# MiguelAlgaba/photoconsistency-visual-odometry

Measured on AMD Instinct MI355X. Metric: frame-pair alignments/sec (640x480, 4-level), higher is better.
Workload: dtype f64

## Files before the change

photoconsistency-visual-odometry_amd/csrc/gn_device.hpp:

```cpp
#pragma once

#include <hip/hip_runtime.h>
#include <hip/hip_fp16.h>

#include "phovo_internal.hpp"

namespace phovo_hip {

namespace {

constexpr int WAVE = 64;
constexpr size_t LDS_LIMIT = 160 * 1024;
constexpr int NRED = 32;
constexpr int RED_VALID = 27;

enum {
  C_X = 0, C_Y, C_Z, C_R01, C_R02, C_R11, C_R12,
  C_T1, C_T2, C_T3, C_T4, C_T5, C_T6, C_T8, C_T11, C_T14, C_T15,
  C_T16, C_T17, C_T24, C_CY, C_SY, C_COUNT
};

enum { CTL_DONE = 0, CTL_FLAGS = 1, CTL_PAIR = 2, CTL_OOW = 3, CTL_COUNT = 4 };

__host__ __device__ constexpr size_t lds_fixed_bytes(int threads)
// ... 399 lines not shown
  s.hi_step_r1 = __double2hiint((double)(step_r + 1));
  return s;
}
__device__ __forceinline__ void rowcol_advance(double &cd, double &rd, const RowColStep &s)
{
  cd += s.step_c;
  const bool wrap = cd >= s.w;
  cd -= __hiloint2double(wrap ? s.hi_w : 0, 0);
  rd += __hiloint2double(wrap ? s.hi_step_r1 : s.hi_step_r, 0);
}

struct RowColFromIndex {
  double inv_w, half_inv_w, w;
};
__device__ __forceinline__ RowColFromIndex make_rowcol_from_index(int W)
{
  RowColFromIndex m;
  m.w = (double)W;
  m.inv_w = uniform_f64(1.0 / m.w);
  m.half_inv_w = 0.5 * m.inv_w;
  return m;
}
__device__ __forceinline__ void rowcol_from_index(double kd, const RowColFromIndex &m, double &cd, double &rd)
{
  rd = trunc(fma(kd, m.inv_w, m.half_inv_w));
  cd = fma(-rd, m.w, kd);
}

__device__ __forceinline__ void rowcol_from_index_floor(double kd, const RowColFromIndex &m, double &cd, double &rd)
{
  rd = floor(fma(kd, m.inv_w, m.half_inv_w));
  cd = fma(-rd, m.w, kd);
}

__device__ __forceinline__ double wave_butterfly(double (&acc)[NRED], int lane)
{
  reduce_stage_swap<32, false>(acc);
  reduce_stage_swap<16, true>(acc);
  reduce_stage<8, 4, 8>(acc, lane);
  reduce_stage<4, 4, 4>(acc, lane);
  reduce_stage<2, 4, 2>(acc, lane);
  return acc[0] + dpp_f64<DPP_QUAD_XOR1>(acc[0]);
}

__device__ __forceinline__ void reduce_wave_to_row(double (&acc)[NRED], int lane, int row, double *s_red)
{
  const double total = wave_butterfly(acc, lane);
  const int idx = ((lane >> 5) & 1) * 16 + ((lane >> 4) & 1) * 8 + ((lane >> 3) & 1) * 4 +
                  ((lane >> 2) & 1) * 2 + ((lane >> 1) & 1);
  if ((lane & 1) == 0) s_red[row * NRED + idx] = total;
}

template <int NROWS>
__device__ __forceinline__ void sum_rows_broadcast(int lane, double *s_red, double (&h)[21], double (&g)[6], int &n_valid)
{
  static_assert(NROWS == 1 || NROWS % 2 == 0, "the rows are summed in two halves");
  if constexpr (NROWS > 1) {
    const int j = lane & (NRED - 1);
    const int w0 = (lane >> 5) * (NROWS / 2);
    double r[NROWS / 2];
#pragma unroll
    for (int w2 = 0; w2 < NROWS / 2; w2++) r[w2] = s_red[(w0 + w2) * NRED + j];
    double v = 0.0;
#pragma unroll
    for (int w2 = 0; w2 < NROWS / 2; w2++) v += r[w2];
    const unsigned vlo = (unsigned)__double2loint(v), vhi = (unsigned)__double2hiint(v);
    const auto lo = __builtin_amdgcn_permlane32_swap(vlo, vlo, false, false);
    const auto hi = __builtin_amdgcn_permlane32_swap(vhi, vhi, false, false);
    v = __hiloint2double((int)hi[0], (int)lo[0]) + __hiloint2double((int)hi[1], (int)lo[1]);
    if (lane < NRED) s_red[lane] = v;
  }
#pragma unroll
  for (int q = 0; q < 21; q++) h[q] = s_red[q];
#pragma unroll
  for (int i = 0; i < 6; i++) g[i] = s_red[21 + i];
  n_valid = (int)s_red[RED_VALID];
}

template <int N>
__device__ __forceinline__ void update_and_terminate(int lane, const double (&step)[N], const double (&g)[N], double *s_state,
                                                     double *s_cst, int *s_ctl, double lambda, int max_iter,
                                                     double min_grad_norm, int iteration, int last_valid, double &last_gnorm)
{
  double st[N];
  bool finite = true;
#pragma unroll
  for (int i = 0; i < N; i++) {
    st[i] = s_state[i] - lambda * step[i];
    finite = finite && finite_f64(st[i]);
  }
  double gn2 = 0.0;
#pragma unroll
  for (int i = 0; i < N; i++) gn2 += g[i] * g[i];
  const double gnorm = sqrt(gn2);
  bool done = false;
  if (iteration + 1 >= max_iter) done = true;
  else if (gnorm < min_grad_norm) done = true;
  if (!finite) done = true;
  if (!done) write_pose_constants(st[0], st[1], st[2], st[3], st[4], st[5], s_cst, lane);
  if (lane == 0) {
#pragma unroll
    for (int i = 0; i < N; i++) s_state[i] = st[i];
    s_ctl[CTL_DONE] = done ? 1 : 0;
    if (!finite) s_ctl[CTL_FLAGS] |= (int)PHOVO_PAIR_NONFINITE;
    if (last_valid < N) s_ctl[CTL_FLAGS] |= (int)PHOVO_PAIR_RANK_DEFICIENT;
  }
  last_gnorm = gnorm;
}

template <int NROWS>
__device__ __forceinline__ void sum_rows_solve_update(int lane, double *s_red, double *s_state, double *s_cst, int *s_ctl,
                                                      double lambda, int max_iter, double min_grad_norm,
                                                      int iteration, double &last_gnorm, int &last_valid)
{
  double h[21], g[6];
  sum_rows_broadcast<NROWS>(lane, s_red, h, g, last_valid);
  double step[6];
  solve6_ldlt(h, g, step);
  update_and_terminate<6>(lane, step, g, s_state, s_cst, s_ctl, lambda, max_iter, min_grad_norm, iteration, last_valid,
                          last_gnorm);
}

template <int NW>
__device__ __forceinline__ void reduce_solve_update(double (&acc)[NRED], int lane, int wave, double *s_red,
                                                    double *s_state, double *s_cst, int *s_ctl,
                                                    double lambda, int max_iter, double min_grad_norm,
                                                    int iteration, double &last_gnorm, int &last_valid)
{
  reduce_wave_to_row(acc, lane, wave, s_red);
  __syncthreads();
  if (wave == 0)
    sum_rows_solve_update<NW>(lane, s_red, s_state, s_cst, s_ctl, lambda, max_iter, min_grad_norm, iteration, last_gnorm,
                              last_valid);
  __syncthreads();
}

__device__ __forceinline__ void add_row(double (&acc)[NRED], const double (&Jw)[6], const double (&J)[6], const double res)
{
  int q = 0;
#pragma unroll
  for (int a = 0; a < 6; a++) {
#pragma unroll
    for (int b = a; b < 6; b++) {
      acc[q] = fma(Jw[a], J[b], acc[q]);
      q++;
    }
  }
#pragma unroll
  for (int a = 0; a < 6; a++) acc[21 + a] = fma(Jw[a], res, acc[21 + a]);
}
__device__ __forceinline__ void add_row(double (&acc)[NRED], const double (&J)[6], const double res) { add_row(acc, J, J, res); }

template <int RCP_STEPS>
__device__ __forceinline__ void analytic_row(const double px, const double py, const double pz, const double gxi, const double gyi,
                                             const double fx, const double fy, const double x, const double y, const double z,
                                             const double t1, const double t2, const double t3, const double t4, const double t5,
                                             const double t6, const double t9, const double t11, const double t14,
                                             const double t15, const double cosy, const double siny, double (&J)[6], double &Zr)
{
  Zr = py * t1 + pz * t2 - px * t3;
  const double t25 = fast_rcp<RCP_STEPS>(z + Zr);
  const double Au = pz * t4 + py * t5 + px * t11;
  const double Bv = fma(py, t6, fma(pz, t9, fma(px, t14, y)));
  J[0] = (gxi * fx) * t25;
  J[1] = (gyi * fy) * t25;
  J[2] = -(J[0] * Au + J[1] * Bv) * t25;
  const double Xr = fma(-px, x, Au);
  const double nYr = y - Bv;
  const double ncx = fma(Zr, J[1], nYr * J[2]);
  const double cyc = fma(Zr, J[0], -(Xr * J[2]));
  J[3] = fma(J[1], Xr, J[0] * nYr);
  J[4] = fma(cosy, cyc, siny * ncx);
  J[5] = fma(-t3, J[3], fma(t14, cyc, -(t15 * ncx)));
}

template <typename Kernel, typename Args>
hipError_t launch_persistent(Kernel kernel, int n_pairs, int cu_count, int wgs_per_cu, int threads, size_t lds_bytes,
                             hipStream_t stream, const Args &args)
{
  const int resident = cu_count * wgs_per_cu;
  const dim3 grid((unsigned)(n_pairs < resident ? n_pairs : resident)), block((unsigned)threads);
  hipLaunchKernelGGL(kernel, grid, block, lds_bytes, stream, args);
  return hipGetLastError();
}

}

}
```

photoconsistency-visual-odometry_amd/csrc/gn_kernels.hip:

```cpp

#include <hip/hip_runtime.h>
#include <hip/hip_fp16.h>

#include <cstdlib>
#include <type_traits>

#include "gn_device.hpp"
#include "phovo_internal.hpp"

namespace phovo_hip {

namespace {

#ifdef PHOVO_TIMELINE
#define PHOVO_TIMELINE_BEGIN const int tl_begin = (int)(wall_clock64() & 0x7fffffffull);
#define PHOVO_TIMELINE_END(rep) { (rep).valid_pixels[15] = tl_begin; (rep).valid_pixels[14] = (int)(wall_clock64() & 0x7fffffffull); (rep).iterations[15] = (int)blockIdx.x; }
#else
#define PHOVO_TIMELINE_BEGIN
#define PHOVO_TIMELINE_END(rep)
#endif

struct LevelLds {
  double *cst;
  double *state;
// ... 75 lines not shown
#define PHOVO_STAMP(i) { const unsigned long long t_ = wall_clock64(); stamp_sum[i] += t_ - stamp_last; stamp_last = t_; }
#else
#define PHOVO_STAMP(i)
#endif
  bool first_trip = true;
  while (true) {
#ifdef PHOVO_PHASE_STAMPS
    stamp_last = wall_clock64();
#endif
    int wv = wave;
    if constexpr (NW > 1) asm volatile("" : "+s"(wv));
    const double fr00 = uniform_f64(s_cst[P_FR00]), fr01 = uniform_f64(s_cst[P_FR01]), fr02 = uniform_f64(s_cst[P_FR02]);
    const double fr10 = uniform_f64(s_cst[P_FR10]), fr11 = uniform_f64(s_cst[P_FR11]), fr12 = uniform_f64(s_cst[P_FR12]);
    const double t1 = uniform_f64(s_cst[P_T1]), t2 = uniform_f64(s_cst[P_T2]), t3 = uniform_f64(s_cst[P_T3]);
    const double cxv = s_cst[P_XF], cyv = s_cst[P_YF], czv = s_cst[P_Z];
    const double oxv = s_cst[P_OXI], oyv = s_cst[P_OYI];

    int owner_tag = 0;
    if constexpr (!OWNER_LDS) {
      const int tg = iteration % OWNER_TAG_PERIOD + 1;
      if (iteration > 0 && tg == 1) {
        for (int kk = n_lds + tid; kk < n; kk += T) g_owner[kk] = -1;
        asm volatile("s_waitcnt vmcnt(0) lgkmcnt(0)" ::: "memory");
        __syncthreads();
      }
      owner_tag = tg << OWNER_TAG_SHIFT;
    }

    int inb_lo = 0, inb_hi = 0;
    int n_rows = 0;
    {
      int k = k0, j = 0;
      PHOVO_ROWCOL_BEGIN
      double pz_next;
      if (PARK && OWNER_LDS && !first_trip && wv < depth_chunks) pz_next = s_i0[k];
      else pz_next = plane_load<TD>(rS, k, oD);
      auto warp_chunk = [&](const double pz, const int chunk, unsigned long long &m_out, int &t_out) {
        PHOVO_ROWCOL_HERE
        const double px = fma(cd, ifx, oxv) * pz;
        const double py = fma(rd, ify, oyv) * pz;
        const double Xf = fma(fr02, pz, fma(fr01, py, fma(fr00, px, cxv)));
        const double Yf = fma(fr12, pz, fma(fr11, py, fma(fr10, px, cyv)));
        const double Z = fma(t2, pz, fma(t1, py, fma(-t3, px, czv)));
        const double iz = fast_rcp(Z);
        const double tc = fma(Xf, iz, ox);
        const double tr = fma(Yf, iz, oy);
        const double half_below = __hiloint2double(0x3fdfffff, (int)0xffffffff);
        const int ri = __double2int_rz(tr + half_below), ci = __double2int_rz(tc + half_below);
        const int lanes_left = n - chunk * WAVE;
        const unsigned long long in_image = lanes_left >= WAVE ? ~0ull : ((1ull << lanes_left) - 1ull);
        const unsigned long long m =
            in_image & __builtin_amdgcn_ballot_w64(min_d < pz) &
            __builtin_amdgcn_ballot_w64(pz < max_d) & __builtin_amdgcn_ballot_w64(tr > -0.5) &
            __builtin_amdgcn_ballot_w64(ri < H) & __builtin_amdgcn_ballot_w64(tc > -0.5) &
            __builtin_amdgcn_ballot_w64(ci < W);
        m_out = m;
        t_out = mad24_uniform_b(ri, W, ci);
      };
      auto keep_mask = [&](const unsigned long long m, const int chunk) {
        if (!MASK_REG) n_rows += __builtin_popcountll(m);
        if (MASK_REG) {
          inb_lo = writelane_b32(inb_lo, (int)(unsigned)m, j);
          inb_hi = writelane_b32(inb_hi, (int)(unsigned)(m >> 32), j);
        } else {
          if (lane == 0) s_mask[chunk] = m;
        }
      };
      if constexpr (OWNER_LDS) {
        auto chunk_body = [&](const int chunk, auto next_parked_tag, auto park_tag) {
          const double pz = pz_next;
          if constexpr (decltype(next_parked_tag)::value) pz_next = s_i0[k + NW * WAVE];
          else pz_next = plane_load<TD>(rS, k + NW * WAVE, oD);
          if constexpr (decltype(park_tag)::value) {
            if (chunk < depth_chunks) s_i0[k] = pz;
          }
          unsigned long long m;
          int t;
          warp_chunk(pz, chunk, m, t);
          if (__builtin_amdgcn_inverse_ballot_w64(m)) atomicMax(&s_owner[t], k);
          keep_mask(m, chunk);
          k += NW * WAVE;
          j++;
          PHOVO_ROWCOL_NEXT
        };
        if (!PARK || first_trip) {
          int chunk = wv;
          for (; chunk + NW < A.n_chunks; chunk += 2 * NW) {
            chunk_body(chunk, std::false_type{}, std::bool_constant<PARK>{});
            chunk_body(chunk + NW, std::false_type{}, std::bool_constant<PARK>{});
          }
          if (chunk < A.n_chunks) chunk_body(chunk, std::false_type{}, std::bool_constant<PARK>{});
        } else {
          const int my_chunks = wv < A.n_chunks ? (A.n_chunks - 1 - wv) / NW + 1 : 0;
          const int parked = depth_chunks > wv ? min(my_chunks, (depth_chunks - 1 - wv) / NW + 1) : 0;
          auto run = [&](int c_lo, int c_end, auto tag) {
            int c = c_lo;
            for (; c + 1 < c_end; c += 2) {
              chunk_body(wv + c * NW, tag, std::false_type{});
              chunk_body(wv + (c + 1) * NW, tag, std::false_type{});
            }
            if (c < c_end) chunk_body(wv + c * NW, tag, std::false_type{});
          };
          if (parked > 0) {
            run(0, parked - 1, std::true_type{});
            chunk_body(wv + (parked - 1) * NW, std::false_type{}, std::false_type{});
          }
          run(parked, my_chunks, std::false_type{});
        }
      } else {
        constexpr int G = 4;
        double pzg[G], pzn[G];
        int pend_t[G], pend_v[G];
        unsigned long long pend_m[G];
        pzg[0] = pz_next;
#pragma unroll
        for (int g = 1; g < G; g++) pzg[g] = plane_load<TD>(rS, k + g * NW * WAVE, oD);
        int chunk = wv;
        while (chunk < A.n_chunks) {
#pragma unroll
          for (int g = 0; g < G; g++) pzn[g] = plane_load<TD>(rS, k + (G + g) * NW * WAVE, oD);
          int count = 0;
#pragma unroll
          for (int g = 0; g < G; g++) {
            if (chunk < A.n_chunks) {
              warp_chunk(pzg[g], chunk, pend_m[g], pend_t[g]);
              pend_v[g] = owner_tag | k;
              keep_mask(pend_m[g], chunk);
              count = g + 1;
              chunk += NW;
              k += NW * WAVE;
              j++;
              PHOVO_ROWCOL_NEXT
            }
          }
#pragma unroll
          for (int g = 0; g < G; g++) {
            if (g < count && __builtin_amdgcn_inverse_ballot_w64(pend_m[g])) {
              if (pend_t[g] < n_lds) atomicMax(&s_owner[pend_t[g]], pend_v[g] & OWNER_INDEX_MASK);
              else atomicMax(&g_owner[pend_t[g]], pend_v[g]);
            }
          }
#pragma unroll
          for (int g = 0; g < G; g++) pzg[g] = pzn[g];
        }
      }
    }
    PHOVO_STAMP(0)
    __syncthreads();
    PHOVO_STAMP(1)

    const double cz = uniform_f64(s_cst[P_Z]), cx = uniform_f64(s_cst[P_X]);
    const double t4 = uniform_f64(s_cst[P_T4]), t5 = uniform_f64(s_cst[P_T5]), t6 = uniform_f64(s_cst[P_T6]);
    const double t8 = uniform_f64(s_cst[P_T8]), t11 = uniform_f64(s_cst[P_T11]), t14 = uniform_f64(s_cst[P_T14]);
    const double t15 = uniform_f64(s_cst[P_T15]);
    const double cosy = uniform_f64(s_cst[P_CY]), siny = uniform_f64(s_cst[P_SY]);
    const double t9 = -t8;

    double acc[NRED];
#pragma unroll
    for (int j = 0; j < NRED; j++) acc[j] = 0.0;

    auto pass2 = [&](auto huber_tag) {
      constexpr bool HUBER = decltype(huber_tag)::value;
      constexpr bool REV = OWNER_LDS;
      const int my_chunks = wv < A.n_chunks ? (A.n_chunks - 1 - wv) / NW + 1 : 0;
      const int first = REV ? my_chunks - 1 : 0;
      const int k_step = REV ? -NW * WAVE : NW * WAVE;
      int k = k0 + first * (NW * WAVE), j = first;
      double kd = kd0 + (double)first * kd_step, cd, rd;
      int o_n = -1;
      double pz_n = 0.0, gx_n = 0.0, gy_n = 0.0, i1_n = 0.0, i0_n = 0.0;
      const double oxv2 = s_cst[P_OXI], oyv2 = s_cst[P_OYI], cyv2 = s_cst[P_Y];
      int o_raw = -1;
      auto owner_request = [&](int kk) {
        o_raw = (kk >= n_lds && kk < n) ? __hip_atomic_load(&g_owner[kk], __ATOMIC_RELAXED, __HIP_MEMORY_SCOPE_AGENT) : -1;
      };
      if (!OWNER_LDS) owner_request(k);
      int o_ahead = -1;
      auto fetch = [&](int kk, auto parked_tag, const bool another_behind) {
        o_n = -1;
        if (OWNER_LDS) {
          o_n = o_ahead;
          o_ahead = -1;
          if (another_behind) {
            const int k2 = kk + k_step;
            o_ahead = s_owner[k2];
            s_owner[k2] = -1;
          }
        } else {
          if (kk < n_lds) {
            o_n = s_owner[kk];
            s_owner[kk] = -1;
          } else {
            o_n = (o_raw & ~OWNER_INDEX_MASK) == owner_tag ? (o_raw & OWNER_INDEX_MASK) : -1;
          }
          owner_request(kk + NW * WAVE);
        }
        if constexpr (decltype(parked_tag)::value) pz_n = s_i0[max(kk, 0)];
        else pz_n = plane_load<TD>(rS, kk, oD);
        gx_n = plane_load<TI>(rT, kk, oGX);
        gy_n = plane_load<TI>(rT, kk, oGY);
        i1_n = plane_load<TI>(rT, kk, oI);
        if (SRC_LDS) { if (o_n >= 0) i0_n = s_i0[o_n]; }
        else i0_n = plane_load<TI>(rS, o_n, oI);
      };
      if (OWNER_LDS && my_chunks > 0) {
        o_ahead = s_owner[k];
        s_owner[k] = -1;
      }
      if (PARK && wv + first * NW < depth_chunks) fetch(k, std::true_type{}, my_chunks >= 2);
      else fetch(k, std::false_type{}, my_chunks >= 2);
      auto chunk_body = [&](const int chunk, auto next_parked_tag, const int behind) {
        const int o = o_n;
        const double pz = pz_n, gxi = gx_n, gyi = gy_n, pixel2 = i1_n, pixel1 = i0_n;
        fetch(k + k_step, next_parked_tag, behind > 0);
        const unsigned long long mbits =
            MASK_REG ? (((unsigned long long)(unsigned)__builtin_amdgcn_readlane(inb_hi, j) << 32) |
                        (unsigned long long)(unsigned)__builtin_amdgcn_readlane(inb_lo, j))
                     : s_mask[chunk];
        if (__builtin_amdgcn_inverse_ballot_w64(mbits)) {
          const double res = (o >= 0) ? (pixel2 - pixel1) : 0.0;
          PHOVO_ROWCOL_HERE
          const double px = fma(cd, ifx, oxv2) * pz;
          const double py = fma(rd, ify, oyv2) * pz;

          double J[6], Zr;
          analytic_row<1>(px, py, pz, gxi, gyi, fx, fy, cx, cyv2, cz, t1, t2, t3, t4, t5, t6, t9, t11, t14, t15, cosy, siny, J, Zr);

          double Jw[6];
#pragma unroll
          for (int a = 0; a < 6; a++) Jw[a] = J[a];
          if (HUBER) {
            const double ar = fabs(res);
            const double wgt = ar <= huber_delta ? 1.0 : huber_delta / ar;
#pragma unroll
            for (int a = 0; a < 6; a++) Jw[a] = J[a] * wgt;
          }
          int q = 0;
#pragma unroll
          for (int a = 0; a < 6; a++) {
#pragma unroll
            for (int b = a; b < 6; b++) {
              acc[q] = fma(Jw[a], J[b], acc[q]);
              q++;
            }
          }
#pragma unroll
          for (int a = 0; a < 6; a++) acc[21 + a] = fma(Jw[a], res, acc[21 + a]);
        }
        k += k_step;
        j += REV ? -1 : 1;
        kd += REV ? -kd_step : kd_step;
      };
      if (REV) {
        auto run = [&](int c_hi, int c_lo, auto tag) {
          for (int c = c_hi; c >= c_lo; c -= 2) {
            chunk_body(wv + c * NW, tag, c - 1);
            if (c > c_lo) chunk_body(wv + (c - 1) * NW, tag, c - 2);
          }
        };
        if (PARK) {
          const int c_split = depth_chunks > wv ? min(my_chunks - 1, (depth_chunks - 1 - wv) / NW + 1) : -1;
          run(my_chunks - 1, c_split + 1, std::false_type{});
          run(min(my_chunks - 1, c_split), 0, std::true_type{});
        } else {
          run(my_chunks - 1, 0, std::false_type{});
        }
      } else {
        for (int chunk = wv; chunk < A.n_chunks; chunk += 2 * NW) {
          chunk_body(chunk, std::false_type{}, 0);
          if (chunk + NW < A.n_chunks) chunk_body(chunk + NW, std::false_type{}, 0);
        }
      }
    };
    if (huber_on) pass2(std::true_type{}); else pass2(std::false_type{});
    PHOVO_STAMP(2)
    acc[RED_VALID] = MASK_REG ? (double)(__popc((unsigned)inb_lo) + __popc((unsigned)inb_hi)) : (lane == 0 ? (double)n_rows : 0.0);


    {
      const double total = wave_butterfly(acc, lane);
      int ln = lane;
      asm volatile("" : "+v"(ln));
      const int idx = ((ln >> 5) & 1) * 16 + ((ln >> 4) & 1) * 8 + ((ln >> 3) & 1) * 4 + ((ln >> 2) & 1) * 2 + ((ln >> 1) & 1);
      if ((ln & 1) == 0) s_red[wave * NRED + idx] = total;
    }
    PHOVO_STAMP(3)
    __syncthreads();
    PHOVO_STAMP(4)

    if (wave == 0) {
      int ln0 = lane;
      asm volatile("" : "+v"(ln0));
      double h[21], g[6];
      sum_rows_broadcast<NW>(ln0, s_red, h, g, last_valid);
#ifdef PHOVO_PHASE_STAMPS
      asm volatile("" :: "v"(h[0]), "v"(g[5]));
      const unsigned long long solve_t0 = wall_clock64();
#endif
      double step[6];
      solve6_ldlt(h, g, step);
#ifdef PHOVO_PHASE_STAMPS
      asm volatile("" :: "v"(step[0]), "v"(step[5]));
      const unsigned long long solve_t1 = wall_clock64();
      solve_sum[0] += solve_t0 - stamp_last;
      solve_sum[1] += solve_t1 - solve_t0;
#endif
      double st[6];
      bool finite = true;
#pragma unroll
      for (int i = 0; i < 6; i++) {
        st[i] = s_state[i] - A.lambda * step[i];
        finite = finite && (fabs(st[i]) <= 1.79769313486231570815e308);
      }
      double gn2 = 0.0;
#pragma unroll
      for (int i = 0; i < 6; i++) gn2 += g[i] * g[i];
      const double gnorm = sqrt(gn2);
      const int it = iteration + 1;
      bool done = false;
      if (it >= A.max_iter) done = true;
      else if (gnorm < A.min_grad_norm) done = true;
      if (!finite) done = true;
#ifdef PHOVO_PHASE_STAMPS
      asm volatile("" :: "v"(gnorm));
      const unsigned long long solve_t2 = wall_clock64();
      solve_sum[2] += solve_t2 - solve_t1;
#endif
      if (!done) write_pass_constants(st[0], st[1], st[2], st[3], st[4], st[5], fx, fy, s_cst, lane);
#ifdef PHOVO_PHASE_STAMPS
      asm volatile("s_waitcnt lgkmcnt(0)" ::: "memory");
      solve_sum[3] += wall_clock64() - solve_t2;
#endif
      if (lane == 0) {
#pragma unroll
        for (int i = 0; i < 6; i++) s_state[i] = st[i];
        s_ctl[CTL_DONE] = done ? 1 : 0;
        if (!finite) s_ctl[CTL_FLAGS] |= (int)PHOVO_PAIR_NONFINITE;
        if (last_valid < 6) s_ctl[CTL_FLAGS] |= (int)PHOVO_PAIR_RANK_DEFICIENT;
      }
      last_gnorm = gnorm;
    }
    __syncthreads();
    PHOVO_STAMP(5)
    iteration++;
    first_trip = false;
    if (s_ctl[CTL_DONE]) break;
  }
#ifdef PHOVO_PHASE_STAMPS
  if (blockIdx.x == 0 && lane == 0 && (wave == 0 || wave == 1 || wave == NW / 2 || wave == NW - 1))
    printf("stamps T=%d level n=%d it=%d wave %2d: pass1 %llu barrier %llu pass2 %llu butterfly %llu barrier %llu solve/wait %llu prologue %llu (10 ns ticks)\n",
           T, n, iteration, wave, stamp_sum[0], stamp_sum[1], stamp_sum[2], stamp_sum[3], stamp_sum[4], stamp_sum[5], stamp_prologue);
  if (blockIdx.x == 0 && lane == 0 && wave == 0)
    printf("stamps T=%d level n=%d it=%d inside wave 0's serial section: row sums %llu  LDL^T %llu  update+norm %llu  pose constants %llu\n",
           T, n, iteration, solve_sum[0], solve_sum[1], solve_sum[2], solve_sum[3]);
#endif
#undef PHOVO_STAMP
#undef PHOVO_ROWCOL_BEGIN
#undef PHOVO_ROWCOL_HERE
#undef PHOVO_ROWCOL_NEXT
}


template <int T, bool SRC_LDS, bool OWNER_LDS, bool MASK_REG>
__device__ __forceinline__ LevelLds carve_lds(unsigned char *lds_raw, int n_max, int n_chunks_max)
{
  constexpr int NW = T / WAVE;
  LevelLds L;
  L.cst = reinterpret_cast<double *>(lds_raw);
  L.state = L.cst + 32;
  L.red = L.state + 8;
  L.ctl = reinterpret_cast<int *>(L.red + NW * NRED);
  L.mask = reinterpret_cast<unsigned long long *>(L.ctl + CTL_COUNT);
  unsigned char *p = reinterpret_cast<unsigned char *>(L.mask + (MASK_REG ? 0 : n_chunks_max));
  L.owner = reinterpret_cast<int *>(p);
  if (OWNER_LDS) p += sizeof(int) * (size_t)owner_lds_entries(n_max, T);
  L.i0 = reinterpret_cast<double *>(p);
  return L;
}

template <int T, int WPS, bool SRC_LDS, bool OWNER_LDS, bool MASK_REG, typename TI, typename TD, bool PARK = false>
__global__ __launch_bounds__(T, WPS) __attribute__((aligned(T == WAVE ? 4096 : 256))) void gn_level_kernel(const GNLevelArgs A)
{
  if constexpr (T == WAVE) asm volatile(".fill 896, 4, 0xbf800000");
  extern __shared__ __align__(16) unsigned char lds_raw[];
  const LevelLds L = carve_lds<T, SRC_LDS, OWNER_LDS, MASK_REG>(lds_raw, A.n, A.g_mask ? 0 : A.n_chunks);
  int *const s_ctl = L.ctl;
  const int tid = threadIdx.x;
  for (int k = tid; k < (OWNER_LDS ? owner_lds_entries(A.n, T) : A.n_lds); k += T) L.owner[k] = -1;
  if (tid == 0) s_ctl[CTL_PAIR] = draw_pair_any(A);
  for (;;) {
    asm volatile("s_waitcnt lgkmcnt(0)" ::: "memory");
    __syncthreads();
    const int pair = __builtin_amdgcn_readfirstlane(s_ctl[CTL_PAIR]);
    if (pair >= A.n_pairs) break;

    int iteration = 0;
    if (A.handover_in) iteration = __builtin_amdgcn_readfirstlane(A.reports[pair].iterations[A.level]);
    double last_gnorm = 0.0;
    int last_valid = 0;
    PHOVO_TIMELINE_BEGIN
    level_body<T, SRC_LDS, OWNER_LDS, MASK_REG, TI, TD, PARK>(A, L, pair, false, iteration, last_gnorm, last_valid);

    if (tid == 0) {
#pragma unroll
      for (int j = 0; j < 6; j++) A.states[(size_t)pair * 6 + j] = L.state[j];
      if (A.reports) {
        A.reports[pair].iterations[A.level] = iteration;
        A.reports[pair].gradient_norm = last_gnorm;
        A.reports[pair].valid_pixels[A.level] = last_valid;
        const uint32_t new_flags = (uint32_t)s_ctl[CTL_FLAGS] | (A.handover_in ? A.takeover_flag : 0u);
        if (new_flags) atomicOr(&A.reports[pair].flags, new_flags);
        PHOVO_TIMELINE_END(A.reports[pair])
      }
      s_ctl[CTL_PAIR] = draw_pair_any(A);
    }
  }
}

template <int T, int WPS, typename TI, typename TD>
__global__ __launch_bounds__(T, WPS) void gn_fused_kernel(const GNFusedArgs F)
{
  extern __shared__ __align__(16) unsigned char lds_raw[];
  const LevelLds L = carve_lds<T, false, true, true>(lds_raw, F.n_max, 0);
  int *const s_ctl = L.ctl;
  const int tid = threadIdx.x;
  for (int k = tid; k < owner_lds_entries(F.n_max, T); k += T) L.owner[k] = -1;
  if (tid == 0) s_ctl[CTL_PAIR] = draw_pair(F.work_counter, F.n_queues, F.n_pairs);
  for (;;) {
    asm volatile("s_waitcnt lgkmcnt(0)" ::: "memory");
    __syncthreads();
    const int pair = __builtin_amdgcn_readfirstlane(s_ctl[CTL_PAIR]);
    if (pair >= F.n_pairs) break;

    double last_gnorm = 0.0;
    PHOVO_TIMELINE_BEGIN
    for (int li = 0; li < F.n_levels; li++) {
      const GNLevelArgs &A = F.lv[li];
      int iteration = 0, last_valid = 0;
      LevelLds Ll = L;
      int *const tail = L.owner + owner_lds_entries(A.n, T);
      Ll.i0 = reinterpret_cast<double *>(tail);
      level_body<T, false, true, true, TI, TD, true>(A, Ll, pair, li > 0, iteration, last_gnorm, last_valid);
      for (int k = tid; k < A.depth_lds_chunks * (int)(WAVE * sizeof(double) / sizeof(int)); k += T) tail[k] = -1;
      if (tid == 0 && A.reports) {
        A.reports[pair].iterations[A.level] = iteration;
        A.reports[pair].valid_pixels[A.level] = last_valid;
      }
    }

    if (tid == 0) {
      const GNLevelArgs &A = F.lv[0];
// ... 201 lines not shown
```

photoconsistency-visual-odometry_amd/csrc/gn_slide_kernel.hip:

```cpp
#include <hip/hip_runtime.h>
#include <hip/hip_fp16.h>

#include <cstdlib>
#include <type_traits>

#include "gn_device.hpp"
#include "phovo_internal.hpp"

namespace phovo_hip {

namespace {

constexpr int SLIDE_RING_PX = 32768;
constexpr int SLIDE_MASK_RING = 512;
static_assert((SLIDE_RING_PX & (SLIDE_RING_PX - 1)) == 0 && (SLIDE_MASK_RING & (SLIDE_MASK_RING - 1)) == 0, "ring indices are masks");

template <int T_, int NW1_, int B1_, int B2_>
struct SlideGeom {
  static constexpr int T = T_, NW = T_ / WAVE, NW1 = NW1_, NW2 = NW - NW1_, B1 = B1_, B2 = B2_;
  static constexpr int BAND_CHUNKS = NW1 * B1;
  static constexpr int BAND_PX = BAND_CHUNKS * WAVE;
  static constexpr int RING_BANDS = SLIDE_RING_PX / BAND_PX;
  static constexpr int M_MAX = (RING_BANDS - 1) / 2;
  static_assert(NW1 * B1 == NW2 * B2, "both kinds of waves cover one band per phase");
  static_assert(NW2 % 2 == 0, "the cross-wave sum splits the rows of s_red in two halves");
  static_assert((M_MAX + 2) * BAND_CHUNKS <= SLIDE_MASK_RING, "ballots of the bands between pass 1 and pass 2");
};

template <int T, int NW1, int B1, int B2, typename TI, typename TD>
__global__ __launch_bounds__(T, T / 256) void gn_level_kernel_slide(const GNLevelArgs A)
{
  using G = SlideGeom<T, NW1, B1, B2>;
  constexpr int NW2 = G::NW2, BAND_CHUNKS = G::BAND_CHUNKS, BAND_PX = G::BAND_PX;
  extern __shared__ __align__(16) unsigned char lds_raw[];
  double *s_cst = reinterpret_cast<double *>(lds_raw);
  double *s_state = s_cst + 32;
  double *s_red = s_state + 8;
  int *s_ctl = reinterpret_cast<int *>(s_red + NW2 * NRED);
  unsigned long long *s_mask = reinterpret_cast<unsigned long long *>(s_ctl + CTL_COUNT);
  int *s_owner = reinterpret_cast<int *>(s_mask + SLIDE_MASK_RING);

  const int tid = threadIdx.x;
  const int lane = tid & (WAVE - 1);
  const int wave = __builtin_amdgcn_readfirstlane(tid / WAVE);
  const int n = A.n, W = A.w, H = A.h;
  const int n_bands = (A.n_chunks + BAND_CHUNKS - 1) / BAND_CHUNKS;
  const int m_run = A.slide_m;
  const int n_phases = n_bands + m_run + 1;
  const int oI = (int)A.plane_off[PLANE_I], oD = (int)A.plane_off[PLANE_D];
  const int oGX = (int)A.plane_off[PLANE_GX], oGY = (int)A.plane_off[PLANE_GY];
  if (tid == 0) s_ctl[CTL_PAIR] = draw_pair(A.work_counter, A.n_queues, A.n_pairs);
  for (;;) {
  asm volatile("s_waitcnt lgkmcnt(0)" ::: "memory");
  __syncthreads();
  const int pair = __builtin_amdgcn_readfirstlane(s_ctl[CTL_PAIR]);
  if (pair >= A.n_pairs) break;

  const __amdgpu_buffer_rsrc_t rS = frame_rsrc(A.planes + (size_t)A.src[pair] * A.frame_bytes, A.frame_bytes);
  const __amdgpu_buffer_rsrc_t rT = frame_rsrc(A.planes + (size_t)A.tgt[pair] * A.frame_bytes, A.frame_bytes);

  for (int k = tid; k < SLIDE_RING_PX; k += T) s_owner[k] = -1;
  if (wave == 0) {
    double st[6];
#pragma unroll
    for (int j = 0; j < 6; j++) st[j] = A.states[(size_t)pair * 6 + j];
    write_pose_constants(st[0], st[1], st[2], st[3], st[4], st[5], s_cst, lane);
    if (lane == 0) {
#pragma unroll
      for (int j = 0; j < 6; j++) s_state[j] = st[j];
      s_ctl[CTL_DONE] = 0;
      s_ctl[CTL_FLAGS] = 0;
      s_ctl[CTL_OOW] = 0;
    }
  }
  __syncthreads();

  const double fx = A.fx, fy = A.fy, ox = A.ox, oy = A.oy, ifx = A.ifx, ify = A.ify;
  const double dW = (double)W;
  const double oxi = uniform_f64(-(ox + 0.5) * ifx), oyi = uniform_f64(-oy * ify);
  const double inv_w = uniform_f64(1.0 / dW);

  int iteration = 0;
  double last_gnorm = 0.0;
  int last_valid = 0;
  bool handed_over = false;
  while (true) {
    if (wave < NW1) {
      const double min_d = A.min_depth, max_d = A.max_depth;
      const double cx = uniform_f64(s_cst[C_X]), cyy = uniform_f64(s_cst[C_Y]), cz = uniform_f64(s_cst[C_Z]);
      const double fr00 = uniform_f64(uniform_f64(s_cst[C_T15]) * fx), fr01 = uniform_f64(uniform_f64(s_cst[C_R01]) * fx);
      const double fr02 = uniform_f64(uniform_f64(s_cst[C_R02]) * fx);
      const double fr10 = uniform_f64(uniform_f64(s_cst[C_T14]) * fy), fr11 = uniform_f64(uniform_f64(s_cst[C_R11]) * fy);
      const double fr12 = uniform_f64(uniform_f64(s_cst[C_R12]) * fy);
      const double t1 = uniform_f64(s_cst[C_T1]), t2 = uniform_f64(s_cst[C_T2]), t3 = uniform_f64(s_cst[C_T3]);
      double cxv = cx * fx, cyv = cyy * fy, czv = cz, oxv = oxi, oyv = oyi;
      asm volatile("" : "+v"(cxv), "+v"(cyv), "+v"(czv), "+v"(oxv), "+v"(oyv));
      const double half_below = __hiloint2double(0x3fdfffff, (int)0xffffffff);
      constexpr int STEP = NW1 * WAVE;
      int k1 = wave * WAVE + lane, chunk1 = wave;
      double kd1 = (double)k1 + 0.5;
      double pzb[B1];
#pragma unroll
      for (int b = 0; b < B1; b++) pzb[b] = plane_load<TD>(rS, k1 + b * STEP, oD);
      for (int s = 0; s < n_bands; s++) {
        const int win_lo = (s - m_run + 1) * BAND_PX;
        const unsigned win_span = (unsigned)(2 * m_run * BAND_PX);
#pragma unroll
        for (int b = 0; b < B1; b++) {
          const double pz = pzb[b];
          pzb[b] = plane_load<TD>(rS, k1 + B1 * STEP, oD);
          const double rd = trunc(kd1 * inv_w), cd = fma(-rd, dW, kd1);
          const double px = fma(cd, ifx, oxv) * pz;
          const double py = fma(rd, ify, oyv) * pz;
          const double Xf = fma(fr02, pz, fma(fr01, py, fma(fr00, px, cxv)));
          const double Yf = fma(fr12, pz, fma(fr11, py, fma(fr10, px, cyv)));
          const double Z = fma(t2, pz, fma(t1, py, fma(-t3, px, czv)));
          const double iz = fast_rcp(Z);
          const double tc = fma(Xf, iz, ox);
          const double tr = fma(Yf, iz, oy);
          const int ri = __double2int_rz(tr + half_below), ci = __double2int_rz(tc + half_below);
          const int lanes_left = n - chunk1 * WAVE;
          const unsigned long long in_image =
              lanes_left >= WAVE ? ~0ull : (lanes_left > 0 ? ((1ull << lanes_left) - 1ull) : 0ull);
          unsigned long long m =
              in_image & __builtin_amdgcn_ballot_w64(min_d < pz) & __builtin_amdgcn_ballot_w64(pz < max_d) &
              __builtin_amdgcn_ballot_w64(tr > -0.5) & __builtin_amdgcn_ballot_w64(ri < H) &
              __builtin_amdgcn_ballot_w64(tc > -0.5) & __builtin_amdgcn_ballot_w64(ci < W);
          const int t = mad24_uniform_b(ri, W, ci);
          const unsigned long long inside = __builtin_amdgcn_ballot_w64((unsigned)(t - win_lo) < win_span);
          if (m & ~inside) {
            if (lane == 0) s_ctl[CTL_OOW] = 1;
            m &= inside;
          }
          if (__builtin_amdgcn_inverse_ballot_w64(m)) atomicMax(&s_owner[t & (SLIDE_RING_PX - 1)], k1);
          if (lane == 0) s_mask[chunk1 & (SLIDE_MASK_RING - 1)] = m;
          k1 += STEP;
          chunk1 += NW1;
          kd1 += (double)STEP;
        }
        __syncthreads();
      }
      for (int s = n_bands; s < n_phases; s++) __syncthreads();
    } else {
      const int wave2 = wave - NW1;
      const double cx = uniform_f64(s_cst[C_X]), cyy = uniform_f64(s_cst[C_Y]), cz = uniform_f64(s_cst[C_Z]);
      const double t1 = uniform_f64(s_cst[C_T1]), t2 = uniform_f64(s_cst[C_T2]), t3 = uniform_f64(s_cst[C_T3]);
      const double t14 = uniform_f64(s_cst[C_T14]);
      const double t4 = uniform_f64(s_cst[C_T4]), t5 = uniform_f64(s_cst[C_T5]), t6 = uniform_f64(s_cst[C_T6]);
      const double t8 = uniform_f64(s_cst[C_T8]), t11 = uniform_f64(s_cst[C_T11]);
      const double t15 = uniform_f64(s_cst[C_T15]);
      const double cosy = uniform_f64(s_cst[C_CY]), siny = uniform_f64(s_cst[C_SY]);
      const double t9 = -t8;
      const double huber_delta = A.huber_delta;
      const bool huber_on = huber_delta > 0.0;
      constexpr int STEP = NW2 * WAVE;

      double acc[NRED];
#pragma unroll
      for (int j = 0; j < NRED; j++) acc[j] = 0.0;
      int n_rows = 0;

      for (int s = 0; s < m_run; s++) __syncthreads();
      int k2 = wave2 * WAVE + lane, chunk2 = wave2;
      double kd2 = (double)k2 + 0.5;
      struct Slots {
        int own[B2];
        double i0[B2], pz[B2], gx[B2], gy[B2], i1[B2];
      };
      Slots set_a, set_b;
      auto request = [&](Slots &S, const int b, const int kk) {
        const int o = s_owner[kk & (SLIDE_RING_PX - 1)];
        s_owner[kk & (SLIDE_RING_PX - 1)] = -1;
        S.own[b] = o;
        S.pz[b] = plane_load<TD>(rS, kk, oD);
        S.gx[b] = plane_load<TI>(rT, kk, oGX);
        S.gy[b] = plane_load<TI>(rT, kk, oGY);
        S.i1[b] = plane_load<TI>(rT, kk, oI);
        S.i0[b] = plane_load<TI>(rS, o, oI);
      };
#pragma unroll
      for (int b = 0; b < B2; b++) request(set_a, b, k2 + b * STEP);
      __syncthreads();

      double oxv2 = oxi, oyv2 = oyi, cyv2 = cyy;
      asm volatile("" : "+v"(oxv2), "+v"(oyv2), "+v"(cyv2));
      auto one_phase = [&](const Slots &cur, Slots &nxt, auto huber_tag) {
        constexpr bool HUBER = decltype(huber_tag)::value;
        {
#pragma unroll
          for (int b = 0; b < B2; b++) {
            const int o = cur.own[b];
            const double pz = cur.pz[b], gxi = cur.gx[b], gyi = cur.gy[b], pixel2 = cur.i1[b], pixel1 = cur.i0[b];
            request(nxt, b, k2 + B2 * STEP);
            const unsigned long long mbits = s_mask[chunk2 & (SLIDE_MASK_RING - 1)];
            const unsigned long long mrow = ((unsigned long long)(unsigned)__builtin_amdgcn_readfirstlane((int)(mbits >> 32)) << 32) |
                                            (unsigned long long)(unsigned)__builtin_amdgcn_readfirstlane((int)mbits);
            n_rows += __builtin_popcountll(mrow);
            if (__builtin_amdgcn_inverse_ballot_w64(mrow)) {
              const double res = (o >= 0) ? (pixel2 - pixel1) : 0.0;
              const double rd = trunc(kd2 * inv_w), cd = fma(-rd, dW, kd2);
              const double px = fma(cd, ifx, oxv2) * pz;
              const double py = fma(rd, ify, oyv2) * pz;
              double J[6], Zr;
              analytic_row<1>(px, py, pz, gxi, gyi, fx, fy, cx, cyv2, cz, t1, t2, t3, t4, t5, t6, t9, t11, t14, t15, cosy, siny, J, Zr);
              double Jw[6];
#pragma unroll
              for (int a = 0; a < 6; a++) Jw[a] = J[a];
              if (HUBER) {
                const double ar = fabs(res);
                const double wgt = ar <= huber_delta ? 1.0 : huber_delta / ar;
#pragma unroll
                for (int a = 0; a < 6; a++) Jw[a] = J[a] * wgt;
              }
              int q = 0;
#pragma unroll
              for (int a = 0; a < 6; a++) {
#pragma unroll
                for (int c = a; c < 6; c++) {
                  acc[q] = fma(Jw[a], J[c], acc[q]);
                  q++;
                }
              }
#pragma unroll
              for (int a = 0; a < 6; a++) acc[21 + a] = fma(Jw[a], res, acc[21 + a]);
            }
            k2 += STEP;
            chunk2 += NW2;
            kd2 += (double)STEP;
          }
          __syncthreads();
        }
      };
      auto run_phases = [&](auto huber_tag) {
        for (int s = m_run + 1; s < n_phases; s += 2) {
          one_phase(set_a, set_b, huber_tag);
          if (s + 1 >= n_phases) break;
          one_phase(set_b, set_a, huber_tag);
        }
      };
      if (huber_on) run_phases(std::true_type{}); else run_phases(std::false_type{});
      acc[RED_VALID] = lane == 0 ? (double)n_rows : 0.0;

      {
        const double total = wave_butterfly(acc, lane);
        const int idx = ((lane >> 5) & 1) * 16 + ((lane >> 4) & 1) * 8 + ((lane >> 3) & 1) * 4 +
                        ((lane >> 2) & 1) * 2 + ((lane >> 1) & 1);
        if ((lane & 1) == 0) s_red[wave2 * NRED + idx] = total;
      }
    }
    __syncthreads();

    if (wave == 0) {
      double h[21], g[6];
      int n_valid;
      sum_rows_broadcast<NW2>(lane, s_red, h, g, n_valid);
      const bool void_iteration = s_ctl[CTL_OOW] != 0;
      double step[6];
      solve6_ldlt(h, g, step);
      double st[6];
      bool finite = true;
#pragma unroll
      for (int i = 0; i < 6; i++) {
        st[i] = s_state[i] - A.lambda * step[i];
        finite = finite && (fabs(st[i]) <= 1.79769313486231570815e308);
      }
      double gn2 = 0.0;
#pragma unroll
      for (int i = 0; i < 6; i++) gn2 += g[i] * g[i];
      const double gnorm = sqrt(gn2);
      const int it = iteration + 1;
      bool done = false;
      if (it >= A.max_iter) done = true;
      else if (gnorm < A.min_grad_norm) done = true;
      if (!finite) done = true;
      if (void_iteration) {
        if (lane == 0) { s_ctl[CTL_DONE] = 2; }
      } else {
        if (!done) write_pose_constants(st[0], st[1], st[2], st[3], st[4], st[5], s_cst, lane);
        if (lane == 0) {
#pragma unroll
          for (int i = 0; i < 6; i++) s_state[i] = st[i];
          s_ctl[CTL_DONE] = done ? 1 : 0;
          if (!finite) s_ctl[CTL_FLAGS] |= (int)PHOVO_PAIR_NONFINITE;
          if (n_valid < 6) s_ctl[CTL_FLAGS] |= (int)PHOVO_PAIR_RANK_DEFICIENT;
        }
        last_gnorm = gnorm;
        last_valid = n_valid;
      }
    }
    __syncthreads();
    const int done_word = s_ctl[CTL_DONE];
    if (done_word == 2) { handed_over = true; break; }
    iteration++;
    if (done_word) break;
  }

  if (tid == 0) {
#pragma unroll
    for (int j = 0; j < 6; j++) A.states[(size_t)pair * 6 + j] = s_state[j];
    if (A.reports) {
      A.reports[pair].iterations[A.level] = iteration;
      A.reports[pair].gradient_norm = last_gnorm;
      A.reports[pair].valid_pixels[A.level] = last_valid;
      A.reports[pair].flags |= (uint32_t)s_ctl[CTL_FLAGS];
    }
    if (handed_over) handover_append(A, pair);
    s_ctl[CTL_PAIR] = draw_pair(A.work_counter, A.n_queues, A.n_pairs);
  }
  }
}

}

#define PHOVO_SLIDE_GEOM 768, 4, 6, 3
using SlideShipped = SlideGeom<PHOVO_SLIDE_GEOM>;

size_t gn_slide_lds_bytes()
{
  return sizeof(double) * (32 + 8 + (size_t)SlideShipped::NW2 * NRED) + sizeof(int) * CTL_COUNT +
         sizeof(unsigned long long) * SLIDE_MASK_RING + sizeof(int) * (size_t)SLIDE_RING_PX;
}

int gn_slide_threads() { return SlideShipped::T; }

int gn_slide_reach_bands(int w, int h)
{
  const int rows = h / 12 > 16 ? h / 12 : 16;
  int m = (rows * w + SlideShipped::BAND_PX - 1) / SlideShipped::BAND_PX + 1;
  if (m > SlideShipped::M_MAX) m = SlideShipped::M_MAX;
  return m < 2 ? 2 : m;
}

hipError_t gn_prepare_slide_kernels()
{
  hipError_t e;
#define PHOVO_PREP_SLIDE(GEOM, TI, TD)                                                                             \
  e = hipFuncSetAttribute(reinterpret_cast<const void *>(&gn_level_kernel_slide<GEOM, TI, TD>),                    \
                          hipFuncAttributeMaxDynamicSharedMemorySize, (int)gn_slide_lds_bytes());                  \
  if (e != hipSuccess) return e;
  PHOVO_PREP_SLIDE(PHOVO_SLIDE_GEOM, double, double)
  PHOVO_PREP_SLIDE(PHOVO_SLIDE_GEOM, float, float)
  PHOVO_PREP_SLIDE(PHOVO_SLIDE_GEOM, __half, float)
#undef PHOVO_PREP_SLIDE
  return hipSuccess;
}

template <int T, int NW1, int B1, int B2>
static hipError_t launch_slide_geom(const GNLevelArgs &a, int storage, int n_blocks, hipStream_t stream)
{
  const dim3 grid((unsigned)n_blocks), block((unsigned)T);
  const size_t lds = gn_slide_lds_bytes();
  switch (storage) {
    case PHOVO_STORAGE_F64: hipLaunchKernelGGL((gn_level_kernel_slide<T, NW1, B1, B2, double, double>), grid, block, lds, stream, a); break;
    case PHOVO_STORAGE_F32: hipLaunchKernelGGL((gn_level_kernel_slide<T, NW1, B1, B2, float, float>), grid, block, lds, stream, a); break;
    case PHOVO_STORAGE_F16: hipLaunchKernelGGL((gn_level_kernel_slide<T, NW1, B1, B2, __half, float>), grid, block, lds, stream, a); break;
    default: return hipErrorInvalidValue;
  }
  return hipGetLastError();
}

hipError_t gn_launch_level_slide(const GNLevelArgs &a, int storage, int cu_count, hipStream_t stream)
{
  if (a.n_pairs <= 0) return hipSuccess;
  if (!a.handover_out || a.handover_in) return hipErrorInvalidValue;
  if (a.slide_m < 1 || a.slide_m > SlideShipped::M_MAX) return hipErrorInvalidValue;
  const int n_blocks = a.n_pairs < cu_count ? a.n_pairs : cu_count;
  return launch_slide_geom<PHOVO_SLIDE_GEOM>(a, storage, n_blocks, stream);
}

}
```

Before: 310,300.

## Accumulate normal equations in twist basis and rotate the 6x6 system once

Per-pixel Jacobian rows are now computed in an unrotated twist basis, which drops the final Euler-angle mixing FMAs for J[4] and J[5] in both the persistent and sliding kernels. The accumulated Hessian and gradient are then transformed once per iteration by a linear change of basis (rotate_system) before the LDLT solve. This moves a small per-pixel arithmetic cost into a single per-iteration 6x6 update and frees a few uniform registers. The trade-off is different floating-point rounding in the normal equations and a correctness risk in the hand-written tri-index transform.

```diff
diff --git a/photoconsistency-visual-odometry_amd/csrc/gn_device.hpp b/photoconsistency-visual-odometry_amd/csrc/gn_device.hpp
--- a/photoconsistency-visual-odometry_amd/csrc/gn_device.hpp
+++ b/photoconsistency-visual-odometry_amd/csrc/gn_device.hpp
@@ -575,26 +575,59 @@
 __device__ __forceinline__ void add_row(double (&acc)[NRED], const double (&J)[6], const double res) { add_row(acc, J, J, res); }
 
 template <int RCP_STEPS>
+__device__ __forceinline__ void analytic_twist_row(const double px, const double py, const double pz, const double gxi,
+                                                   const double gyi, const double fx, const double fy, const double x,
+                                                   const double y, const double z, const double t1, const double t2,
+                                                   const double t3, const double t4, const double t5, const double t6,
+                                                   const double t9, const double t11, const double t14, double (&q)[6],
+                                                   double &Zr)
+{
+  Zr = py * t1 + pz * t2 - px * t3;
+  const double t25 = fast_rcp<RCP_STEPS>(z + Zr);
+  const double Au = pz * t4 + py * t5 + px * t11;
+  const double Bv = fma(py, t6, fma(pz, t9, fma(px, t14, y)));
+  q[0] = (gxi * fx) * t25;
+  q[1] = (gyi * fy) * t25;
+  q[2] = -(q[0] * Au + q[1] * Bv) * t25;
+  const double Xr = fma(-px, x, Au);
+  const double nYr = y - Bv;
+  q[5] = fma(Zr, q[1], nYr * q[2]);
+  q[4] = fma(Zr, q[0], -(Xr * q[2]));
+  q[3] = fma(q[1], Xr, q[0] * nYr);
+}
+
+template <int RCP_STEPS>
 __device__ __forceinline__ void analytic_row(const double px, const double py, const double pz, const double gxi, const double gyi,
                                              const double fx, const double fy, const double x, const double y, const double z,
                                              const double t1, const double t2, const double t3, const double t4, const double t5,
                                              const double t6, const double t9, const double t11, const double t14,
                                              const double t15, const double cosy, const double siny, double (&J)[6], double &Zr)
 {
-  Zr = py * t1 + pz * t2 - px * t3;
-  const double t25 = fast_rcp<RCP_STEPS>(z + Zr);
-  const double Au = pz * t4 + py * t5 + px * t11;
-  const double Bv = fma(py, t6, fma(pz, t9, fma(px, t14, y)));
-  J[0] = (gxi * fx) * t25;
-  J[1] = (gyi * fy) * t25;
-  J[2] = -(J[0] * Au + J[1] * Bv) * t25;
-  const double Xr = fma(-px, x, Au);
-  const double nYr = y - Bv;
-  const double ncx = fma(Zr, J[1], nYr * J[2]);
-  const double cyc = fma(Zr, J[0], -(Xr * J[2]));
-  J[3] = fma(J[1], Xr, J[0] * nYr);
+  analytic_twist_row<RCP_STEPS>(px, py, pz, gxi, gyi, fx, fy, x, y, z, t1, t2, t3, t4, t5, t6, t9, t11, t14, J, Zr);
+  const double cyc = J[4], ncx = J[5];
   J[4] = fma(cosy, cyc, siny * ncx);
   J[5] = fma(-t3, J[3], fma(t14, cyc, -(t15 * ncx)));
+}
+
+__device__ __forceinline__ void rotate_system(double (&h)[21], double (&g)[6], const double cosy, const double siny,
+                                              const double t3, const double t14, const double t15)
+{
+  auto two = [&](const double a, const double b) { return fma(cosy, a, siny * b); };
+  auto three = [&](const double a, const double b, const double c) { return fma(-t3, a, fma(t14, b, -(t15 * c))); };
+  const double bu4 = two(h[tri(4, 4)], h[tri(4, 5)]), bu5 = two(h[tri(4, 5)], h[tri(5, 5)]);
+  const double bv4 = three(h[tri(3, 4)], h[tri(4, 4)], h[tri(4, 5)]), bv5 = three(h[tri(3, 5)], h[tri(4, 5)], h[tri(5, 5)]);
+#pragma unroll
+  for (int i = 0; i < 4; i++) {
+    const double a3 = h[tri(i, 3)], a4 = h[tri(i, 4)], a5 = h[tri(i, 5)];
+    h[tri(i, 4)] = two(a4, a5);
+    h[tri(i, 5)] = three(a3, a4, a5);
+  }
+  h[tri(4, 4)] = two(bu4, bu5);
+  h[tri(4, 5)] = two(bv4, bv5);
+  h[tri(5, 5)] = three(h[tri(3, 5)], bv4, bv5);
+  const double g3 = g[3], g4 = g[4], g5 = g[5];
+  g[4] = two(g4, g5);
+  g[5] = three(g3, g4, g5);
 }
 
 template <typename Kernel, typename Args>
diff --git a/photoconsistency-visual-odometry_amd/csrc/gn_kernels.hip b/photoconsistency-visual-odometry_amd/csrc/gn_kernels.hip
--- a/photoconsistency-visual-odometry_amd/csrc/gn_kernels.hip
+++ b/photoconsistency-visual-odometry_amd/csrc/gn_kernels.hip
@@ -251,8 +251,6 @@
     const double cz = uniform_f64(s_cst[P_Z]), cx = uniform_f64(s_cst[P_X]);
     const double t4 = uniform_f64(s_cst[P_T4]), t5 = uniform_f64(s_cst[P_T5]), t6 = uniform_f64(s_cst[P_T6]);
     const double t8 = uniform_f64(s_cst[P_T8]), t11 = uniform_f64(s_cst[P_T11]), t14 = uniform_f64(s_cst[P_T14]);
-    const double t15 = uniform_f64(s_cst[P_T15]);
-    const double cosy = uniform_f64(s_cst[P_CY]), siny = uniform_f64(s_cst[P_SY]);
     const double t9 = -t8;
 
     double acc[NRED];
@@ -324,7 +322,7 @@
           const double py = fma(rd, ify, oyv2) * pz;
 
           double J[6], Zr;
-          analytic_row<1>(px, py, pz, gxi, gyi, fx, fy, cx, cyv2, cz, t1, t2, t3, t4, t5, t6, t9, t11, t14, t15, cosy, siny, J, Zr);
+          analytic_twist_row<1>(px, py, pz, gxi, gyi, fx, fy, cx, cyv2, cz, t1, t2, t3, t4, t5, t6, t9, t11, t14, J, Zr);
 
           double Jw[6];
 #pragma unroll
@@ -393,10 +391,13 @@
       asm volatile("" : "+v"(ln0));
       double h[21], g[6];
       sum_rows_broadcast<NW>(ln0, s_red, h, g, last_valid);
+      const double rot_cy = uniform_f64(s_cst[P_CY]), rot_sy = uniform_f64(s_cst[P_SY]), rot_t3 = uniform_f64(s_cst[P_T3]);
+      const double rot_t14 = uniform_f64(s_cst[P_T14]), rot_t15 = uniform_f64(s_cst[P_T15]);
 #ifdef PHOVO_PHASE_STAMPS
       asm volatile("" :: "v"(h[0]), "v"(g[5]));
       const unsigned long long solve_t0 = wall_clock64();
 #endif
+      rotate_system(h, g, rot_cy, rot_sy, rot_t3, rot_t14, rot_t15);
       double step[6];
       solve6_ldlt(h, g, step);
 #ifdef PHOVO_PHASE_STAMPS
diff --git a/photoconsistency-visual-odometry_amd/csrc/gn_slide_kernel.hip b/photoconsistency-visual-odometry_amd/csrc/gn_slide_kernel.hip
--- a/photoconsistency-visual-odometry_amd/csrc/gn_slide_kernel.hip
+++ b/photoconsistency-visual-odometry_amd/csrc/gn_slide_kernel.hip
@@ -148,8 +148,6 @@
       const double t14 = uniform_f64(s_cst[C_T14]);
       const double t4 = uniform_f64(s_cst[C_T4]), t5 = uniform_f64(s_cst[C_T5]), t6 = uniform_f64(s_cst[C_T6]);
       const double t8 = uniform_f64(s_cst[C_T8]), t11 = uniform_f64(s_cst[C_T11]);
-      const double t15 = uniform_f64(s_cst[C_T15]);
-      const double cosy = uniform_f64(s_cst[C_CY]), siny = uniform_f64(s_cst[C_SY]);
       const double t9 = -t8;
       const double huber_delta = A.huber_delta;
       const bool huber_on = huber_delta > 0.0;
@@ -202,7 +200,7 @@
               const double px = fma(cd, ifx, oxv2) * pz;
               const double py = fma(rd, ify, oyv2) * pz;
               double J[6], Zr;
-              analytic_row<1>(px, py, pz, gxi, gyi, fx, fy, cx, cyv2, cz, t1, t2, t3, t4, t5, t6, t9, t11, t14, t15, cosy, siny, J, Zr);
+              analytic_twist_row<1>(px, py, pz, gxi, gyi, fx, fy, cx, cyv2, cz, t1, t2, t3, t4, t5, t6, t9, t11, t14, J, Zr);
               double Jw[6];
 #pragma unroll
               for (int a = 0; a < 6; a++) Jw[a] = J[a];
@@ -251,10 +249,12 @@
     __syncthreads();
 
     if (wave == 0) {
+      const double rot_cy = s_cst[C_CY], rot_sy = s_cst[C_SY], rot_t3 = s_cst[C_T3], rot_t14 = s_cst[C_T14], rot_t15 = s_cst[C_T15];
       double h[21], g[6];
       int n_valid;
       sum_rows_broadcast<NW2>(lane, s_red, h, g, n_valid);
       const bool void_iteration = s_ctl[CTL_OOW] != 0;
+      rotate_system(h, g, rot_cy, rot_sy, rot_t3, rot_t14, rot_t15);
       double step[6];
       solve6_ldlt(h, g, step);
       double st[6];
```

Result: faster. 315,400 (median of 6 runs) (+1.6%).
